# grospy/bitcoincashplus

Measured on AMD Instinct MI355X. Metric: equihash_200_9_solutions_per_sec, higher is better.
Workload: dtype uint32; 1 GPU; model=Equihash(200,9) mainnet PoW solver (BLAKE2b, K=9 collision rounds), global_batch=96, seq_len=2097152, parallelism=dp1 (nonce-space), solvers_in_flight=2, full=False, verified_solutions=0, gpu_cpu_verifier_disagreements=0, rows_dropped_all_nonces=231487, pairs_dropped_all_nonces=346475, candidates_dropped_all_nonces=0

## Files before the change

csrc/kernels/equihash_layout.h:

```cpp
#ifndef BCP_KERNELS_EQUIHASH_LAYOUT_H
#define BCP_KERNELS_EQUIHASH_LAYOUT_H

#include <cstddef>
#include <cstdint>
#include <stdexcept>

#if defined(__HIPCC__)
#define BCP_EH_HD __host__ __device__
#else
#define BCP_EH_HD
#endif

#ifndef BCP_EH_GEN_HPT
#define BCP_EH_GEN_HPT 2
#endif
#ifndef BCP_EH_GEN_NT
#define BCP_EH_GEN_NT 512
#endif
#ifndef BCP_EH_PRUNE_FROM
#define BCP_EH_PRUNE_FROM 9
#endif
#ifndef BCP_EH_MP_LATE
#define BCP_EH_MP_LATE 1
#endif
// ... 17 lines not shown
static_assert(BCP_EH_OVL >= 1 && BCP_EH_OVL <= 128, "the overflow list is walked by the first BCP_EH_OVL lanes");

namespace bcpk {

template <class C> constexpr int round_nt(int stage, bool carry);
template <class C> constexpr int round_mp(int stage, bool carry = false);
template <class C> constexpr bool round_prunes(int stage, bool carry = false);
template <class C> constexpr bool slot_round_fits(int stage);

template <int N_, int K_, int BB_, int CAP_, int NT_, int GENWG_, int NTG_, int MAXCAND_, int CAP4_ = CAP_,
          int CAP3_ = CAP_, int WGCU_ = 1, int GNT_ = 512, int GHPT_ = 2, int CAPF_ = 0, int MPX_ = 0, int GW_ = 0>
struct EhCfg {
    static constexpr int N = N_, K = K_;
    static constexpr int DB = N / (K + 1);
    static constexpr int BB = BB_;
    static constexpr int RB = DB - BB_;
    static constexpr int NB = 1 << BB_;
    static constexpr int NRESTS = 1 << RB;
    static constexpr int CAP = CAP_;
    static constexpr int CAPF = CAPF_ > 0 ? CAPF_ : CAP3_;
    static constexpr int MPX = MPX_;
    static constexpr int cap(int round) {
        return round == K_ ? CAPF : words(round - 1) >= 5 ? CAP_ : words(round - 1) == 4 ? CAP4_ : CAP3_;
    }
    static constexpr int AREA_NF = CAP_ > CAP4_ ? (CAP_ > CAP3_ ? CAP_ : CAP3_) : (CAP4_ > CAP3_ ? CAP4_ : CAP3_);
    static constexpr int AREA = AREA_NF > CAPF ? AREA_NF : CAPF;
    static constexpr int NT = NT_;
    static constexpr int NW = NT_ / 64;
    static constexpr int GW = GW_;
    static constexpr int RNT = NT_ - 64 * GW_;
    static constexpr int WGCU = WGCU_;
    static constexpr int LDS_BUDGET = 160 * 1024 / WGCU_;
    static constexpr int INIT = 1 << (DB + 1);
    static constexpr int GENWG = GENWG_;
    static constexpr int NTG = NTG_;
    static constexpr int GNT = GNT_, GHPT = GHPT_;
    static constexpr int RPW = INIT / GENWG_;
    static constexpr int IPH = 512 / N;
    static constexpr int NBYTES = N / 8;
    static constexpr int MAXCAND = MAXCAND_;
    static constexpr int L = 1 << K;
    static constexpr int bits(int stage) { return N - stage * DB - BB_; }
    static constexpr int words(int stage) { return (bits(stage) + 31) / 32; }
    static constexpr int WMAX = words(0);
    static constexpr int IB = AREA <= 4096 ? 12 : 13;
    static constexpr int DH = 16 - IB;
    static constexpr uint32_t DHM = (1u << DH) - 1;
    static constexpr int DX = 2 * DH;
    static constexpr int DR = BB_ > DX ? BB_ - DX : 0;
    static constexpr uint32_t RMASK = (1u << DR) - 1;
    static constexpr uint32_t IMASK = ((1u << IB) - 1) * 0x10001u;
    static constexpr bool cp(int stage) {
        return stage >= 1 && stage < K && 32 * words(stage) - bits(stage) >= DR;
    }
    static constexpr int pad(int stage) { return 32 * words(stage) - bits(stage); }
    static constexpr bool tp(int stage) {
        return BCP_EH_TABLE_PARENTS && stage >= 1 && stage <= K - 2 && !round_prunes<EhCfg>(stage + 1) &&
               !round_prunes<EhCfg>(stage + 1, true) && pad(stage) >= BB;
    }
    static constexpr int ptab(int stage) {
        const int a = round_mp<EhCfg>(stage, false) * round_nt<EhCfg>(stage, false);
        const int b = GW_ > 0 ? round_mp<EhCfg>(stage, true) * round_nt<EhCfg>(stage, true) : 0;
        return a > b ? a : b;
    }
    static constexpr uint32_t tpmask(int stage) { return (1u << (pad(stage) > BB ? BB + 1 : BB)) - 1; }
    static constexpr uint32_t rmask(int stage) { return tp(stage) ? (uint32_t)NB - 1 : cp(stage) ? RMASK : 0u; }
    static constexpr int sw(int stage) {
        return stage == 0 || tp(stage) ? words(stage) : words(stage) + (cp(stage) ? 1 : 2);
    }
    static constexpr size_t ROWS = (size_t)NB * AREA;
    static constexpr int ks(int stage) {
        return BCP_EH_KEY_SLOTS && stage >= 1 && stage < K && NRESTS >= 256 && slot_round_fits<EhCfg>(stage)
                   ? BCP_EH_KEY_SLOTS
                   : 0;
    }
    static constexpr int PDW = 2 * K + 2 + (BCP_EH_KEY_SLOTS ? 2 * K : 0);
    static constexpr bool H16 = NB > 512;
    static constexpr int HW = H16 ? NB / 2 : NB;
    static_assert(RPW * GENWG_ == INIT && RPW < 65535, "generation split");
    static_assert(RB > 0 && DB < 32, "digit geometry");
    static_assert(AREA < (1 << IB), "LDS row indices in parent words and signatures");
    static_assert(NT_ % 64 == 0 && NT_ <= 1024 && (NB <= NT_ || NB % NT_ == 0) && NB <= NTG_ && NT_ / 64 <= 64,
                  "workgroup shape");
    static_assert(words(K - 1) == 1, "final round keeps whole rows in one LDS word");
    static_assert(GW_ == 0 || (WGCU_ == 1 && RNT >= 128 && (NB <= RNT || NB % RNT == 0)), "carrying workgroup shape");
};

#ifndef BCP_EH_CAPF
#define BCP_EH_CAPF 6016
#endif
using Cfg200_9 = EhCfg<200, 9, 9, 4416, 1024, 512, 1024, 256, 4864, 5120, 1, BCP_EH_GEN_NT, BCP_EH_GEN_HPT, BCP_EH_CAPF, 0, BCP_EH_GW>;
using Cfg96_5 = EhCfg<96, 5, 7, 1280, 256, 256, 256, 256, 1280, 1280, 1, 512, 2, 0, 1, 1>;
using Cfg48_5 = EhCfg<48, 5, 3, 512, 64, 8, 64, 256>;

constexpr uint32_t NIL = 0xffffffffu;

template <class C, int NTG, int HPT> struct GenReg {
    static constexpr int RPT = HPT * C::IPH;
    static constexpr int RPW = NTG > 0 ? NTG * RPT : 1;
    static constexpr bool OK = NTG > 0 && C::INIT % RPW == 0;
    static constexpr int GWG = OK ? C::INIT / RPW : 1;
};

BCP_EH_HD inline __attribute__((always_inline)) uint64_t pack_tri(uint32_t d, uint32_t i, uint32_t j) {
    return ((uint64_t)d << 32) | (j << 16) | i;
}
template <class C> BCP_EH_HD inline __attribute__((always_inline)) uint32_t cpack(uint32_t d, uint32_t i, uint32_t j) {
    return i | (j << 16) | ((d & C::DHM) << C::IB) | (((d >> C::DH) & C::DHM) << (16 + C::IB));
}
template <class C> BCP_EH_HD inline __attribute__((always_inline)) uint32_t cunpack_d(uint32_t pw, uint32_t lastword) {
    return ((pw >> C::IB) & C::DHM) | (((pw >> (16 + C::IB)) & C::DHM) << C::DH) | ((lastword & C::RMASK) << C::DX);
}

template <class C> constexpr int un_walk_bend(int cap) { return (cap * 2 + 3) / 4 * 4; }
template <class C> constexpr int un_walk_list(int cap) { return un_walk_bend<C>(cap) + C::NRESTS * 4; }
template <class C> constexpr int round_nt(int stage, bool carry) { return carry && stage < C::K ? C::RNT : C::NT; }
template <class C> constexpr int round_mp(int stage, bool carry) {
    const int nt = round_nt<C>(stage, carry);
    return stage == C::K ? 1
                         : (C::AREA_NF + nt - 1) / nt + C::MPX +
                               (C::K == 9 && stage >= BCP_EH_MP_LATE_FROM ? BCP_EH_MP_LATE : 0);
}
template <class C> constexpr int round_un(int stage, bool carry = false) {
    const int cap = C::cap(stage);
    if (stage == C::K) return un_walk_list<C>(cap);
    const int pairs = round_mp<C>(stage, carry) * round_nt<C>(stage, carry) * 4;
    const int walk = un_walk_list<C>(cap) + pairs;
    return walk > pairs ? walk : pairs;
}
template <class C> constexpr int round_lds(int stage, bool prune, bool carry = false) {
    const int WR = C::words(stage - 1);
    const int WI = WR;
    const int cap = C::cap(stage);
    const int pruneb = prune ? cap * 4 + (C::cp(stage - 1) ? 0 : (cap * 2 + 3) / 4 * 4) : 0;
    const int hists = stage == C::K ? 0 : 2 * C::HW * 4 + (C::NB * (C::H16 ? 2 : 4) + 3) / 4 * 4;
    const int gen = carry ? 2 * C::NB * 4 + 16 * 8 : 0;
    return (cap * WI + 3) / 4 * 16 + pruneb + 4 + round_un<C>(stage, carry) + hists +
           (round_nt<C>(stage, carry) / 64 + 1) * 4 + gen;
}
template <class C> constexpr int un_slot_bend() { return C::NRESTS * 8 * 2; }
template <class C> constexpr int un_slot_ovl() { return un_slot_bend<C>() + C::NRESTS * 4; }
template <class C> constexpr int un_slot_list() { return un_slot_ovl<C>() + BCP_EH_OVL * 4; }
template <class C> constexpr int slot_un(int stage, bool carry = false) {
    return un_slot_list<C>() + round_mp<C>(stage, carry) * round_nt<C>(stage, carry) * 4;
}
template <class C> constexpr int slot_lds(int stage, bool prune, bool carry = false) {
    const int b = round_lds<C>(stage, prune, carry) - round_un<C>(stage, carry) + slot_un<C>(stage, carry) + 4;
    return carry ? (b + 7) / 8 * 8 : b;
}
struct EhBars {
    int n, list, filter, scan, sort;
};
constexpr EhBars eh_bars(bool slot) { return slot ? EhBars{7, 2, 3, 4, 6} : EhBars{10, 5, 6, 7, 9}; }
template <class C> constexpr bool round_prunes(int stage, bool carry) {
    constexpr int from = C::K == 9 ? BCP_EH_PRUNE_FROM : 2;
    return (stage >= from || stage == C::K) && stage >= 2 && round_lds<C>(stage, true, carry) <= C::LDS_BUDGET;
}

template <class C> constexpr bool slot_round_fits(int stage) {
    return slot_lds<C>(stage, round_prunes<C>(stage, false), false) <= C::LDS_BUDGET &&
           (C::GW == 0 || slot_lds<C>(stage, round_prunes<C>(stage, true), true) <= C::LDS_BUDGET);
}

template <class C> struct GenCarry {
    static constexpr int GT = C::GW > 0 ? 64 * C::GW : 64;
    static constexpr int NHASH = (C::INIT + C::IPH - 1) / C::IPH;
    static constexpr int ITERS = (C::K - 1) * C::NB;
    static constexpr int HB = ((NHASH + ITERS - 1) / ITERS + GT - 1) / GT;
    static constexpr int CH = HB * GT;
    static constexpr int RPT = HB * C::IPH;
    static constexpr int BPT = (C::NB + GT - 1) / GT;
    static_assert((long long)CH * ITERS >= NHASH, "the carrying rounds cover every hash");
};

template <class C> BCP_EH_HD inline uint64_t slot_parent(int stage, const uint32_t* slot) {
    const uint32_t* q = slot + C::words(stage);
    if (C::cp(stage)) return ((uint64_t)cunpack_d<C>(q[0], q[-1]) << 32) | (q[0] & C::IMASK);
    return ((uint64_t)q[1] << 32) | q[0];
}
template <class C>
BCP_EH_HD inline uint64_t table_parent(int stage, const uint32_t* row, uint32_t area, uint32_t pos,
                                       const uint32_t* btab_of_nonce, const uint32_t* ptab_of_nonce, bool* in_range) {
    const uint32_t d = row[C::words(stage) - 1] & C::tpmask(stage);
    const uint32_t o = d < (uint32_t)C::NB ? pos - btab_of_nonce[(size_t)d * C::NB + area] : NIL;
    *in_range = d < (uint32_t)C::NB && o < (uint32_t)C::ptab(stage);
    return ((uint64_t)d << 32) | (*in_range ? ptab_of_nonce[(size_t)d * C::ptab(stage) + o] : NIL);
}

}

namespace bcp {
namespace gpu {

template <class F> static void dispatch_cfg(unsigned n, unsigned k, F&& f) {
    if (n == 200 && k == 9) f(bcpk::Cfg200_9{});
    else if (n == 96 && k == 5) f(bcpk::Cfg96_5{});
    else if (n == 48 && k == 5) f(bcpk::Cfg48_5{});
    else throw std::invalid_argument("EquihashGpuSolver: unsupported (N,K); GPU supports (200,9),(96,5),(48,5)");
}

}
}

#endif
```

csrc/kernels/equihash_solver.hip:

```cpp
#include <hip/hip_runtime.h>

#include "crypto/hashes.h"
#include "kernels/blake2b_device.h"
#include "kernels/equihash_layout.h"
#include "kernels/equihash_pow.h"
#include "kernels/gpu_api.h"
#include "kernels/hip_util.h"

#include <algorithm>
#include <cstdlib>
#include <cstring>
#include <stdexcept>
#include <utility>

#ifndef BCP_EH_XCD_MAP
#define BCP_EH_XCD_MAP 1
#endif
#ifndef BCP_EH_PF_SLICES
#define BCP_EH_PF_SLICES 3
#endif
#ifndef BCP_EH_SLOT_LIST
#define BCP_EH_SLOT_LIST 1
#endif
#ifndef BCP_EH_SLOT_RB
#define BCP_EH_SLOT_RB 5
#endif
#ifndef BCP_EH_SLOT_RD
#define BCP_EH_SLOT_RD 10
#endif
#ifndef BCP_EH_GROUPS_DEFAULT
#define BCP_EH_GROUPS_DEFAULT(batch) ((batch) >= 48 ? (batch) / 24 : 1)
#endif

namespace bcpk {

constexpr uint32_t OOB = 0x80000000u;
typedef uint32_t u2v __attribute__((ext_vector_type(2)));
typedef uint32_t u3v __attribute__((ext_vector_type(3)));
typedef uint32_t u4v __attribute__((ext_vector_type(4)));

template <int CTRL, int ROWMASK = 0xf>
__device__ __forceinline__ uint32_t dpp0(uint32_t x) {
    return (uint32_t)__builtin_amdgcn_update_dpp(0, (int)x, CTRL, ROWMASK, 0xf, false);
}
template <bool MAX> __device__ __forceinline__ uint32_t wave_incl(uint32_t x) {
    auto op = [](uint32_t a, uint32_t b) -> uint32_t { return MAX ? (a > b ? a : b) : a + b; };
    x = op(x, dpp0<0x111>(x));
    x = op(x, dpp0<0x112>(x));
    x = op(x, dpp0<0x114>(x));
    x = op(x, dpp0<0x118>(x));
    x = op(x, dpp0<0x142, 0xa>(x));
    x = op(x, dpp0<0x143, 0xc>(x));
    return x;
}

template <int NT, int MAXPER = 4, class TS = uint32_t, class TD = TS>
__device__ uint32_t block_exscan(const TS* src, TD* dst, int n, uint32_t* wsum, uint32_t* mine = nullptr) {
    constexpr int NW = NT / 64;
    const int tid = threadIdx.x, lane = tid & 63;
    const int wid = __builtin_amdgcn_readfirstlane(tid >> 6);
    const int per = (n + NT - 1) / NT;
    uint32_t local[MAXPER];
    uint32_t s = 0;
#pragma unroll
    for (int q = 0; q < MAXPER; ++q) {
        const int i = tid * per + q;
        local[q] = (q < per && i < n) ? (uint32_t)src[i] : 0u;
        s += local[q];
    }
    const uint32_t x = wave_incl<false>(s);
    if (NW > 1) {
        if (lane == 63) wsum[wid] = x;
        __syncthreads();
    }
    const uint32_t wt = (NW > 1 && lane < NW) ? wsum[lane] : 0u;
    const uint32_t ws = wave_incl<false>(wt);
    const uint32_t before = NW > 1 ? __builtin_amdgcn_readlane(ws, wid) - __builtin_amdgcn_readlane(wt, wid) : 0u;
    const uint32_t total = NW > 1 ? __builtin_amdgcn_readlane(ws, NW - 1) : __builtin_amdgcn_readlane(x, 63);
    uint32_t base = before + x - s;
    if (mine) *mine = base;
#pragma unroll
    for (int q = 0; q < MAXPER; ++q) {
        const int i = tid * per + q;
        if (q < per && i < n) dst[i] = (TD)base;
        base += local[q];
    }
    __syncthreads();
    return total;
}
template <int NT, int MAXPER = 4, class T = uint32_t>
__device__ uint32_t block_exscan(T* v, int n, uint32_t* wsum) {
    return block_exscan<NT, MAXPER, T, T>(v, v, n, wsum);
}

template <int NT, int MAXPER = 4, class T = uint32_t>
__device__ void block_maxscan(T* v, int n, uint32_t* wsum) {
    constexpr int NW = NT / 64;
    const int tid = threadIdx.x, lane = tid & 63;
    const int wid = __builtin_amdgcn_readfirstlane(tid >> 6);
    const int per = (n + NT - 1) / NT;
    uint32_t local[MAXPER];
    uint32_t s = 0;
#pragma unroll
    for (int q = 0; q < MAXPER; ++q) {
        const int i = tid * per + q;
        local[q] = (q < per && i < n) ? (uint32_t)v[i] : 0u;
        s = max(s, local[q]);
    }
    const uint32_t x = wave_incl<true>(s);
    const uint32_t excl = dpp0<0x138>(x);
    if (NW > 1) {
        if (lane == 63) wsum[wid] = x;
        __syncthreads();
    }
    const uint32_t wt = (NW > 1 && lane < NW) ? wsum[lane] : 0u;
    const uint32_t ws = wave_incl<true>(wt);
    const uint32_t before = (NW > 1 && wid > 0) ? __builtin_amdgcn_readlane(ws, wid - 1) : 0u;
    uint32_t run = max(before, excl);
#pragma unroll
    for (int q = 0; q < MAXPER; ++q) {
        const int i = tid * per + q;
        run = max(run, local[q]);
        if (q < per && i < n) v[i] = (T)run;
    }
    __syncthreads();
}

template <int W> __device__ __forceinline__ void row_store(__amdgpu_buffer_rsrc_t rs, uint32_t off, const uint32_t* v) {
    if constexpr (W >= 4) {
        const u4v x = {v[0], v[1], v[2], v[3]};
        __builtin_amdgcn_raw_buffer_store_b128(x, rs, off, 0, 0);
        row_store<W - 4>(rs, off + 16, v + 4);
    } else if constexpr (W == 3) {
        const u3v x = {v[0], v[1], v[2]};
        __builtin_amdgcn_raw_buffer_store_b96(x, rs, off, 0, 0);
    } else if constexpr (W == 2) {
        const u2v x = {v[0], v[1]};
        __builtin_amdgcn_raw_buffer_store_b64(x, rs, off, 0, 0);
    } else if constexpr (W == 1) {
        __builtin_amdgcn_raw_buffer_store_b32(v[0], rs, off, 0, 0);
    }
}

template <int W> __device__ __forceinline__ void row_load(__amdgpu_buffer_rsrc_t rs, uint32_t off, uint32_t* v) {
    if constexpr (W >= 4) {
        const u4v x = __builtin_amdgcn_raw_buffer_load_b128(rs, off, 0, 0);
        v[0] = x.x, v[1] = x.y, v[2] = x.z, v[3] = x.w;
        row_load<W - 4>(rs, off + 16, v + 4);
    } else if constexpr (W == 3) {
        const u3v x = __builtin_amdgcn_raw_buffer_load_b96(rs, off, 0, 0);
        v[0] = x.x, v[1] = x.y, v[2] = x.z;
    } else if constexpr (W == 2) {
        const u2v x = __builtin_amdgcn_raw_buffer_load_b64(rs, off, 0, 0);
        v[0] = x.x, v[1] = x.y;
    } else if constexpr (W == 1) {
        v[0] = __builtin_amdgcn_raw_buffer_load_b32(rs, off, 0, 0);
    }
}

template <int WI> __device__ __forceinline__ void lds_row_xor(const uint32_t* rows, uint32_t i, uint32_t j, uint32_t* x) {
    if constexpr (WI % 2 == 0) {
        const u2v* r2 = reinterpret_cast<const u2v*>(rows);
#pragma unroll
        for (int w = 0; w < WI / 2; ++w) {
            const u2v a = r2[i * (WI / 2) + w], b = r2[j * (WI / 2) + w];
            x[2 * w] = a.x ^ b.x;
            x[2 * w + 1] = a.y ^ b.y;
        }
    } else {
#pragma unroll
        for (int w = 0; w < WI; ++w) x[w] = rows[i * WI + w] ^ rows[j * WI + w];
    }
}

__device__ __forceinline__ __amdgpu_buffer_rsrc_t buf_rsrc(const void* p, uint32_t bytes) {
    return __builtin_amdgcn_make_buffer_rsrc(const_cast<void*>(p), 0, bytes, 0x00020000);
}

constexpr int NXCD = 8;
template <int NB> __device__ __forceinline__ int xcd_bucket(int b, int it, int G, int nbk) {
    const int nonces = nbk / NB;
// ... 64 lines not shown
    const auto rs = buf_rsrc(R + (size_t)nonce * C::ROWS * SW0, (uint32_t)(C::ROWS * SW0 * 4));
    uint32_t* leaf = LEAF + (size_t)nonce * C::ROWS;
    for (int t = tid; t < C::RPW; t += NTG) {
        const uint32_t li = perm[t], d = dst[li];
        const uint32_t pos = base[d] + (uint32_t)t;
        if (pos < OCAP) {
            uint32_t o[W0];
#pragma unroll
            for (int w = 0; w < W0; ++w) o[w] = rows[li * W0 + w];
            const uint32_t slot = d * C::AREA + pos;
            row_store<SW0>(rs, slot * (SW0 * 4), o);
            leaf[slot] = r0 + li;
        }
    }
}

template <class C, bool HDR, int NTG, int HPT>
__global__ __launch_bounds__(NTG) __attribute__((amdgpu_waves_per_eu(1))) void eh_gen_reg(const EhBaseState* __restrict__ states, uint32_t* __restrict__ R,
                                                  uint32_t* __restrict__ LEAF, uint32_t* __restrict__ CTR0, int items) {
    using G = GenReg<C, NTG, HPT>;
    static_assert(G::OK, "register generation geometry");
    constexpr int W0 = C::words(0);
    constexpr int SW = (C::N + 31) / 32 + 1;
    constexpr uint32_t OCAP = C::cap(1);
    __shared__ uint32_t hist[C::NB], base[C::NB];
    __shared__ uint64_t r0p[HDR ? 16 : 1];
    const int tid = threadIdx.x;
    for (int b = blockIdx.x; b < items; b += gridDim.x) {
    int gw = b % G::GWG;
    int nonce = b / G::GWG;
    if (BCP_EH_XCD_MAP && (items / G::GWG) % NXCD == 0 && gridDim.x % NXCD == 0) {
        const int x = b % NXCD, j = b / NXCD;
        gw = j % G::GWG;
        nonce = x + NXCD * (j / G::GWG);
    }
    if (b != (int)blockIdx.x) __syncthreads();
    const EhBaseState& bs = states[nonce];
    for (int i = tid; i < C::NB; i += NTG) hist[i] = 0;
    if constexpr (HDR) {
        if (tid == 0) {
            uint64_t P[16];
            eh_hdr_round0_uniform(bs, P);
#pragma unroll
            for (int i = 0; i < 16; ++i) r0p[i] = P[i];
        }
    }
    __syncthreads();
    const uint32_t r0 = (uint32_t)gw * G::RPW;
    const uint32_t g0 = r0 / C::IPH;
    uint32_t rw[G::RPT][W0];
    uint32_t rk[G::RPT];
#pragma unroll
    for (int hh = 0; hh < HPT; ++hh) {
        const uint32_t g = g0 + hh * NTG + tid;
        uint64_t h[8];
        if constexpr (HDR) {
            uint64_t P[16];
#pragma unroll
            for (int i = 0; i < 16; ++i) P[i] = r0p[i];
            eh_hash_g_hdr_from(P, bs, g, h);
        } else {
            eh_hash_g(bs, g, h);
        }
#pragma unroll
        for (int s = 0; s < C::IPH; ++s) {
            uint32_t S[SW];
#pragma unroll
            for (int w = 0; w < SW; ++w) {
                uint32_t v = 0;
#pragma unroll
                for (int t = 0; t < 4; ++t) {
                    const int k = 4 * w + t;
                    v = (v << 8) | ((k < C::NBYTES) ? digest_byte(h, s * C::NBYTES + k) : 0u);
                }
                S[w] = v;
            }
            const int q = hh * C::IPH + s;
            const uint32_t d = S[0] >> (32 - C::BB);
#pragma unroll
            for (int w = 0; w < W0; ++w) rw[q][w] = (S[w] << C::BB) | (S[w + 1] >> (32 - C::BB));
            rk[q] = (atomicAdd(&hist[d], 1u) << 16) | d;
        }
    }
    __syncthreads();
    for (int b = tid; b < C::NB; b += NTG) {
        const uint32_t c = hist[b];
        base[b] = c ? atomicAdd(&CTR0[(size_t)nonce * C::NB + b], c) : 0u;
    }
    __syncthreads();
    constexpr int SW0 = C::sw(0);
    const auto rs = buf_rsrc(R + (size_t)nonce * C::ROWS * SW0, (uint32_t)(C::ROWS * SW0 * 4));
    const auto rl = buf_rsrc(LEAF + (size_t)nonce * C::ROWS, (uint32_t)(C::ROWS * 4));
#pragma unroll
    for (int q = 0; q < G::RPT; ++q) {
        const uint32_t d = rk[q] & 0xffff;
        const uint32_t pos = base[d] + (rk[q] >> 16);
        const uint32_t slot = d * C::AREA + pos;
        const bool ok = pos < OCAP;
        const uint32_t g = g0 + (q / C::IPH) * NTG + tid;
        const uint32_t li = g * C::IPH + (q % C::IPH);
        row_store<W0>(rs, ok ? slot * (SW0 * 4) : OOB, rw[q]);
        __builtin_amdgcn_raw_buffer_store_b32(li, rl, ok ? slot * 4 : OOB, 0, 0);
    }
    }
}

#define EH_STAMP(k)                                                                                  \
    do {                                                                                             \
        if constexpr (STAMP) {                                                                       \
            if (threadIdx.x == 0) stamps[(size_t)bk * 16 + (k)] = __builtin_amdgcn_s_memtime();        \
        }                                                                                            \
    } while (0)

struct EhCarry {
    const EhBaseState* states;
    uint32_t* R0;
    uint32_t* LEAF;
    uint32_t* CTR0;
    int nonces;
};

constexpr int EH_SCAN_BARS = 2;
template <int K, int NBAR> __device__ __forceinline__ void eh_bar() {
    static_assert(K >= 1 && K <= NBAR, "barrier outside the bucket iteration's count");
    __syncthreads();
}
#define EH_BAR_SCAN(k, nbar) static_assert((k) >= 1 && (k) + EH_SCAN_BARS - 1 <= (nbar), "scan barriers")

template <class C, int STAGE>
__device__ __forceinline__ void eh_carry_gen(const EhCarry& cy, int nbk, uint32_t* ghist, uint32_t* gbase, uint64_t* gr0p) {
    using GC = GenCarry<C>;
    constexpr int W0 = C::words(0);
    constexpr int SW = (C::N + 31) / 32 + 1;
    constexpr int SW0 = C::sw(0);
    constexpr int GT = GC::GT, HB = GC::HB;
    constexpr uint32_t OCAP = C::cap(1);
    const int gtid = (int)threadIdx.x - C::RNT;
    const int G = gridDim.x;
    auto chunk_of = [&](int b) -> int {
        const int nonce = b / C::NB, c = (STAGE - 1) * C::NB + b % C::NB;
        return (nonce < cy.nonces && (long long)c * GC::CH < GC::NHASH) ? c : -1;
    };
    auto prefix = [&](int b) {
        if (gtid == 0 && b / C::NB < cy.nonces) {
            uint64_t P[16];
            eh_hdr_round0_uniform(cy.states[b / C::NB], P);
#pragma unroll
            for (int i = 0; i < 16; ++i) gr0p[i] = P[i];
        }
    };
    constexpr bool SLOT = C::ks(STAGE) > 0;
    constexpr EhBars BAR = eh_bars(SLOT);
    constexpr int NBAR = BAR.n;
    constexpr int RA = 3, RB = SLOT ? BCP_EH_SLOT_RB : 5, RC = SLOT ? RB : 6, RD = SLOT ? BCP_EH_SLOT_RD : 10;
    static_assert(RA <= RB && RB <= RC && RC <= RD && RD <= 12, "BLAKE2b slices in order");
    EhHdrHash hs[HB];
    auto start = [&](int b) {
        const int c = chunk_of(b);
        if (c < 0) return;
        const EhBaseState& bs = cy.states[b / C::NB];
        uint64_t P[16];
#pragma unroll
        for (int i = 0; i < 16; ++i) P[i] = gr0p[i];
#pragma unroll
        for (int hh = 0; hh < HB; ++hh) {
            hs[hh].begin(P, bs, (uint32_t)c * GC::CH + (uint32_t)(hh * GT + gtid));
            hs[hh].template rounds<1, RA>(bs);
        }
    };
    int it = 0;
    int bk = xcd_bucket<C::NB>(blockIdx.x, 0, G, nbk);
    for (int i = gtid; i < C::NB; i += GT) ghist[i] = 0;
    prefix(bk);
    __syncthreads();
    start(bk);
    for (;;) {
        const int nonce = bk / C::NB;
        const int chunk = chunk_of(bk);
        const bool act = chunk >= 0;
        const EhBaseState& bs = cy.states[act ? nonce : 0];
        const int bn = xcd_bucket<C::NB>(blockIdx.x, it + 1, G, nbk);
        const bool more = bn >= 0;
        const uint32_t g0 = (uint32_t)chunk * GC::CH + (uint32_t)gtid;
        uint32_t rw[GC::RPT][W0];
        uint32_t rk[GC::RPT];
        uint32_t myb[GC::BPT];
        if (act) {
#pragma unroll
            for (int hh = 0; hh < HB; ++hh) hs[hh].template rounds<RA, RB>(bs);
        }
        eh_bar<1, NBAR>();
        if constexpr (!SLOT) {
            eh_bar<2, NBAR>();
            eh_bar<3, NBAR>();
            if (act) {
#pragma unroll
                for (int hh = 0; hh < HB; ++hh) hs[hh].template rounds<RB, RC>(bs);
            }
            eh_bar<4, NBAR>();
        }
        if (act) {
#pragma unroll
            for (int hh = 0; hh < HB; ++hh) hs[hh].template rounds<RC, RD>(bs);
        }
        if (more && bn / C::NB != nonce) prefix(bn);
        eh_bar<BAR.list, NBAR>();
        if (act) {
#pragma unroll
            for (int hh = 0; hh < HB; ++hh) {
                hs[hh].template rounds<RD, 12>(bs);
                uint64_t h[8];
                hs[hh].finish(bs, h);
                const uint32_t g = g0 + hh * GT;
#pragma unroll
                for (int s = 0; s < C::IPH; ++s) {
                    uint32_t S[SW];
#pragma unroll
                    for (int w = 0; w < SW; ++w) {
                        uint32_t v = 0;
#pragma unroll
                        for (int t = 0; t < 4; ++t) {
                            const int k = 4 * w + t;
                            v = (v << 8) | ((k < C::NBYTES) ? digest_byte(h, s * C::NBYTES + k) : 0u);
                        }
                        S[w] = v;
                    }
                    const int q = hh * C::IPH + s;
                    const uint32_t d = S[0] >> (32 - C::BB);
#pragma unroll
                    for (int w = 0; w < W0; ++w) rw[q][w] = (S[w] << C::BB) | (S[w + 1] >> (32 - C::BB));
                    rk[q] = NIL;
                    if (g * C::IPH + s < (uint32_t)C::INIT) rk[q] = (atomicAdd(&ghist[d], 1u) << 16) | d;
                }
            }
        }
        eh_bar<BAR.filter, NBAR>();
        if (act) {
#pragma unroll
            for (int k = 0; k < GC::BPT; ++k) {
                const int b = gtid + k * GT;
                const uint32_t c = b < C::NB ? ghist[b] : 0u;
                myb[k] = 0;
                if (c) myb[k] = atomicAdd(&cy.CTR0[(size_t)nonce * C::NB + b], c);
            }
        }
        eh_bar<BAR.scan, NBAR>();
        if (act)
            for (int i = gtid; i < C::NB; i += GT) ghist[i] = 0;
        eh_bar<BAR.scan + 1, NBAR>();
        if (act) {
#pragma unroll
            for (int k = 0; k < GC::BPT; ++k) {
                const int b = gtid + k * GT;
                if (b < C::NB) gbase[b] = myb[k];
            }
        }
        eh_bar<BAR.sort, NBAR>();
        if (act) {
            const auto rs = buf_rsrc(cy.R0 + (size_t)nonce * C::ROWS * SW0, (uint32_t)(C::ROWS * SW0 * 4));
            const auto rl = buf_rsrc(cy.LEAF + (size_t)nonce * C::ROWS, (uint32_t)(C::ROWS * 4));
#pragma unroll
            for (int q = 0; q < GC::RPT; ++q) {
                const uint32_t d = rk[q] & 0xffff;
                const uint32_t pos = gbase[d < (uint32_t)C::NB ? d : 0] + (rk[q] >> 16);
                const uint32_t slot = d * C::AREA + pos;
                const bool ok = rk[q] != NIL && pos < OCAP;
                const uint32_t li = (g0 + (q / C::IPH) * GT) * C::IPH + (q % C::IPH);
                row_store<W0>(rs, ok ? slot * (SW0 * 4) : OOB, rw[q]);
                __builtin_amdgcn_raw_buffer_store_b32(li, rl, ok ? slot * 4 : OOB, 0, 0);
            }
        }
        if (more) start(bn);
        eh_bar<NBAR, NBAR>();
        if (!more) break;
        bk = bn;
        ++it;
    }
}

template <class C, int STAGE, bool STAMP, bool CARRY = false>
__global__ __launch_bounds__(C::NT) __attribute__((amdgpu_waves_per_eu(C::WGCU * C::NT / 256)))
void eh_round(const uint32_t* __restrict__ Rin, const uint32_t* __restrict__ CTRin, uint32_t* __restrict__ Rout,
              uint32_t* __restrict__ CTRout, uint32_t* __restrict__ Pout, uint32_t* __restrict__ Bout,
              uint32_t* __restrict__ ncand, uint64_t* __restrict__ cand, uint64_t* __restrict__ stamps,
              uint32_t* __restrict__ pdrop, int nbk, EhCarry carry) {
    constexpr int WI = C::words(STAGE - 1);
    constexpr int WO = (STAGE < C::K) ? C::words(STAGE) : 1;
    constexpr int CAP = C::cap(STAGE);
    constexpr bool FINAL = STAGE == C::K;
    constexpr int PDW = C::PDW;
    static_assert(!CARRY || (C::GW > 0 && !FINAL && !STAMP), "only plain collision rounds carry generation");
    constexpr bool PRUNE = round_prunes<C>(STAGE, CARRY);
    static_assert(PRUNE == round_prunes<C>(STAGE), "a carrying round prunes like the plain one");
    constexpr bool SLOT = C::ks(STAGE) > 0;
    constexpr EhBars BAR = eh_bars(SLOT);
    constexpr int NBAR = BAR.n;
    constexpr int OVL = BCP_EH_OVL;
    static_assert((SLOT ? slot_lds<C>(STAGE, PRUNE, CARRY) : round_lds<C>(STAGE, PRUNE, CARRY)) <= 160 * 1024 / C::WGCU,
                  "round LDS budget");
    constexpr int NT = round_nt<C>(STAGE, CARRY);
    static_assert(!CARRY || NT / 64 > 1, "block_exscan runs its two barriers only with more than one wave");
    constexpr int RPL = (CAP + NT - 1) / NT;
    constexpr int MP = round_mp<C>(STAGE, CARRY);
    constexpr int SWI = C::sw(STAGE - 1);
    constexpr int SWO = STAGE < C::K ? C::sw(STAGE) : 1;
    constexpr bool TPO = !FINAL && C::tp(STAGE);
    constexpr int PTW = TPO ? C::ptab(STAGE) : 1;
// ... 137 lines not shown
        return __builtin_amdgcn_raw_buffer_load_b32(ctr_rs, b >= 0 ? (uint32_t)b * 4 : OOB, 0, 0);
    };

    for (;;) {
        const int nonce = bk / C::NB, d = bk % C::NB;
        EH_STAMP(0);
        if (tid == 0 && fill > (uint32_t)CAP) atomicAdd(&pdrop[nonce * PDW + C::K + STAGE], fill - CAP);
        {
            const uint32_t ot = opaque_tid();
#pragma unroll
            for (int u = 0; u < RPL; ++u) {
                const uint32_t r = ot + u * NT;
                if (r < n) {
                    if constexpr (WI % 2 == 0) {
#pragma unroll
                        for (int w = 0; w < WI; w += 2)
                            *reinterpret_cast<u2v*>(&rows[r * WI + w]) = u2v{nr[u][w], nr[u][w + 1]};
                    } else {
#pragma unroll
                        for (int w = 0; w < WI; ++w) rows[r * WI + w] = nr[u][w];
                    }
                    if constexpr (PRUNE) {
                        psig[r] = nr[u][WI];
                        if constexpr (!CPI) pdw[r] = (uint16_t)nr[u][WI + 1];
                    }
                    if constexpr (FOLD) {
                        const uint32_t key = nr[u][0] >> (32 - C::RB);
                        krank[u] = (key << 16) | atomicAdd(&bend[key], 1u);
                    }
                }
            }
            if constexpr (SLOT) {
#pragma unroll
                for (int u = 0; u < RPL; ++u) {
                    const uint32_t r = ot + u * NT;
                    if (r < n) {
                        const uint32_t key = krank[u] >> 16, t = krank[u] & 0xffff;
                        if (t < 8u) {
                            ktab[key * 8 + t] = (uint16_t)r;
                        } else {
                            const uint32_t o = atomicAdd(&novf, 1u);
                            if (o < (uint32_t)OVL) ovl[o] = (key << 16) | r;
                            krank[u] |= o < (uint32_t)OVL ? 0x4000u : 0x8000u;
                        }
                    }
                }
            }
        }
        if constexpr (!FINAL)
            for (int b = tid; b < C::HW; b += NT) hist_[b] = 0;
        if constexpr (!FOLD)
            for (int k = tid; k < C::NRESTS; k += NT) bend[k] = 0;
        if (tid == 0) npairs = 0;
        EH_STAMP(1);
        const int bn = xcd_bucket<C::NB>(blockIdx.x, it + 1, G, nbk);
        const bool more = bn >= 0;
        const uint32_t fn = more ? (uint32_t)__builtin_amdgcn_readfirstlane(fill_next) : 0u;
        const uint32_t nn = min(fn, (uint32_t)CAP);
        pf_bk = more ? bn : bk;
        pf_n = nn;
        const int bn2 = xcd_bucket<C::NB>(blockIdx.x, it + 2, G, nbk);
        issue(0, SLI);
        fill_next = fill_of(bn2);
        eh_bar<1, NBAR>();
        EH_STAMP(2);

        auto key_of = [&](uint32_t i) -> uint32_t { return rows[i * WI] >> (32 - C::RB); };
        uint32_t kpairs[FOLD ? RPL : 1];
        if constexpr (SLOT) {
            if constexpr (STAMP) {
                if (threadIdx.x == 0) stamps[(size_t)bk * 16 + 3] = stamps[(size_t)bk * 16 + 2];
            }
            issue(SLI, 2 * SLI);
        } else if constexpr (FOLD) {
            EH_BAR_SCAN(2, NBAR);
            block_exscan<NT, (C::NRESTS + NT - 1) / NT>(bend, C::NRESTS, wsum);
            const uint32_t ot = opaque_tid();
#pragma unroll
            for (int u = 0; u < RPL; ++u) {
                const uint32_t r = ot + u * NT;
                kpairs[u] = 0;
                if (r < n) {
                    const uint32_t key = krank[u] >> 16;
                    const uint32_t pos = bend[key] + (krank[u] & 0xffff);
                    const uint32_t e = key + 1 < (uint32_t)C::NRESTS ? bend[key + 1] : n;
                    sidx[pos] = (uint16_t)r;
                    krank[u] = pos;
                    kpairs[u] = min(e - pos - 1, 14u);
                    if (e - pos - 1 > 14u) atomicAdd(&pdrop[nonce * PDW + STAGE], e - pos - 1 - 14u);
                }
            }
        } else {
            for (uint32_t i = tid; i < n; i += NT) atomicAdd(&bend[key_of(i)], 1u);
            __syncthreads();
            block_exscan<NT, (C::NRESTS + NT - 1) / NT>(bend, C::NRESTS, wsum);
            for (uint32_t i = tid; i < n; i += NT) sidx[atomicAdd(&bend[key_of(i)], 1u)] = (uint16_t)i;
        }
        if constexpr (!SLOT) {
            issue(SLI, 2 * SLI);
            eh_bar<4, NBAR>();
            EH_STAMP(3);
        }

        if constexpr (FINAL) {
            static_assert(WI == 1, "final-round rows are one word");
            for (uint32_t p = tid; p < n; p += NT) {
                const uint32_t i = sidx[p], ri = rows[i], e = bend[ri >> (32 - C::RB)];
                for (uint32_t q = p + 1; q < e; ++q) {
                    const uint32_t j = sidx[q];
                    if ((rows[j] ^ ri) & ~RMI) continue;
                    if constexpr (PRUNE) {
                        if (shares_parent(i, j)) continue;
                    }
                    const uint32_t c = atomicAdd(&ncand[nonce], 1u);
                    if (c < (uint32_t)C::MAXCAND) cand[(size_t)nonce * C::MAXCAND + c] = pack_tri(d, i, j);
                }
            }
            issue(2 * SLI, RPL);
        } else {
            uint32_t cnt = 0;
            uint32_t le = 0, lm = 0, ln = 0;
            if constexpr (SLOT) {
                const uint32_t nov = __builtin_amdgcn_readfirstlane(novf);
                const uint32_t NO = min(nov, (uint32_t)OVL);
                const bool full = nov > (uint32_t)OVL;
                ovf_sum += nov;
                ovf_max = max(ovf_max, nov);
#pragma unroll
                for (int u = 0; u < RPL; ++u) {
                    kpairs[u] = 0;
                    if (tid + u * NT < n) {
                        const uint32_t t = krank[u] & 0x3fffu, f = krank[u] & 0xc000u;
                        kpairs[u] = f == 0x4000u ? 0u : min(t, 8u);
                        if (full && f) atomicAdd(&pdrop[nonce * PDW + STAGE], t - 8u);
                    }
                }
                if ((uint32_t)tid < NO) {
                    le = ovl[tid];
                    uint32_t m = 0;
                    for (uint32_t q = 0; q < (uint32_t)tid; ++q) m += (ovl[q] >> 16) == (le >> 16) ? 1u : 0u;
                    lm = min(m, 6u);
                    if (full) {
                        if (lm) atomicSub(&pdrop[nonce * PDW + STAGE], lm);
                    } else if (m > 6u) {
                        atomicAdd(&pdrop[nonce * PDW + STAGE], m - 6u);
                    }
                    ln = 8u + lm;
                    cnt = ln;
                }
            }
#pragma unroll
            for (int u = 0; u < RPL; ++u) cnt += kpairs[u];
            const uint32_t incl = wave_incl<false>(cnt);
            uint32_t wb = 0;
            if ((tid & 63) == 63) wb = atomicAdd(&npairs, incl);
            uint32_t o = __builtin_amdgcn_readlane(wb, 63) + incl - cnt;
            if constexpr (SLOT) {
                auto table_pairs = [&](uint32_t key, uint32_t c, uint32_t i) {
                    const u4v w = *reinterpret_cast<const u4v*>(&ktab[key * 8]);
                    const uint32_t room = o < (uint32_t)(MP * NT) ? (uint32_t)(MP * NT) - o : 0u;
                    const uint32_t ce = min(c, room);
                    if constexpr (BCP_EH_SLOT_LIST == 1) {
                        for (uint32_t q = 0; q < ce; ++q) {
                            const uint32_t ww = q < 4 ? (q < 2 ? w.x : w.y) : (q < 6 ? w.z : w.w);
                            plist[o + q] = ((q & 1) ? (ww & 0xffff0000u) : (ww << 16)) | i;
                        }
                    } else {
#pragma unroll
                        for (int q = 0; q < 8; ++q)
                            if ((uint32_t)q < ce) plist[o + q] = ((q & 1) ? (w[q >> 1] & 0xffff0000u) : (w[q >> 1] << 16)) | i;
                    }
                    o += c;
                };
#pragma unroll
                for (int u = 0; u < RPL; ++u)
                    if (kpairs[u]) table_pairs(krank[u] >> 16, kpairs[u], tid + u * NT);
                if (ln) {
                    const uint32_t i = le & 0xffffu;
                    table_pairs(le >> 16, 8u, i);
                    for (uint32_t q = 0, k = 0; q < (uint32_t)tid && k < lm; ++q) {
                        const uint32_t e = ovl[q];
                        if ((e >> 16) != (le >> 16)) continue;
                        if (o < (uint32_t)(MP * NT)) plist[o] = (e << 16) | i;
                        ++o, ++k;
                    }
                }
            } else {
#pragma unroll
            for (int u = 0; u < RPL; ++u) {
                if (!kpairs[u]) continue;
                const uint32_t p = krank[u];
                const uint32_t i = tid + u * NT;
                for (uint32_t q = p + 1; q <= p + kpairs[u]; ++q, ++o) {
                    if (o >= (uint32_t)(MP * NT)) continue;
                    plist[o] = ((uint32_t)sidx[q] << 16) | i;
                }
            }
            }
            eh_bar<BAR.list, NBAR>();
            EH_STAMP(7);
            const uint32_t P = npairs;
            const uint32_t Pc = min(P, (uint32_t)(MP * NT));
            if (tid == 0 && P > (uint32_t)(MP * NT)) atomicAdd(&pdrop[nonce * PDW + STAGE], P - MP * NT);
            uint32_t pv[MP], pd[MP];
#pragma unroll
            for (int u = 0; u < MP; ++u) {
                const uint32_t k = tid + u * NT;
                pv[u] = NIL;
                pd[u] = 0;
                if (k < Pc) {
                    const uint32_t pr = plist[k];
                    const uint32_t i = pr & 0xffff, j = pr >> 16;
                    uint32_t dest;
                    if (pair_keep(i, j, dest)) {
                        pv[u] = (j << 16) | i;
                        pd[u] = dest;
                        hinc(hist_, pd[u]);
                    }
                }
            }
            for (int k = tid; k < C::NRESTS; k += NT) bend[k] = 0;
            if constexpr (SLOT) {
                if (tid == 0) novf = 0;
            }
            eh_bar<BAR.filter, NBAR>();
            EH_STAMP(4);
            uint32_t myb[BPT];
#pragma unroll
            for (int k = 0; k < BPT; ++k) {
                const int b = tid * BPT + k;
                myb[k] = 0;
                if (b < C::NB) myb[k] = atomicAdd(&CTRout[(size_t)nonce * C::NB + b], hget(hist_, b));
            }
            issue(2 * SLI, RPL);
            uint32_t start = 0;
            uint32_t np;
            EH_BAR_SCAN(BAR.scan, NBAR);
            if constexpr (C::H16)
                np = block_exscan<NT, BPT, uint16_t, uint16_t>(reinterpret_cast<const uint16_t*>(hist_),
                                                               reinterpret_cast<uint16_t*>(cur_), C::NB, wsum, &start);
            else
                np = block_exscan<NT, BPT>(hist_, cur_, C::NB, wsum, &start);
#pragma unroll
            for (int u = 0; u < MP; ++u)
                if (pv[u] != NIL) spair[hinc(cur_, pd[u])] = pv[u];
#pragma unroll
            for (int k = 0; k < BPT; ++k) {
                const int b = tid * BPT + k;
                const uint32_t rb = myb[k] - start;
                if (b < C::NB) {
                    base[b] = (HT)rb;
                    start += hget(hist_, b);
                }
                if constexpr (TPO) {
                    const auto rs_b = buf_rsrc(Bout + ((size_t)nonce * C::NB + d) * C::NB, C::NB * 4);
                    __builtin_amdgcn_raw_buffer_store_b32(rb, rs_b, b < C::NB ? (uint32_t)b * 4 : OOB, 0, 0);
                }
            }
            eh_bar<BAR.sort, NBAR>();
            EH_STAMP(5);
            constexpr uint32_t OCAP = C::cap(STAGE + 1 <= C::K ? STAGE + 1 : C::K);
            constexpr uint32_t RMO = C::rmask(STAGE);
            const auto rs_out = buf_rsrc(Rout + (size_t)nonce * C::ROWS * SWO, (uint32_t)(C::ROWS * SWO * 4));
            const auto rs_p = buf_rsrc(Pout + (TPO ? ((size_t)nonce * C::NB + d) * PTW : 0), TPO ? PTW * 4 : 0);
#pragma unroll
            for (int u = 0; u < MP; ++u) {
                const uint32_t t = tid + u * NT;
                const uint32_t pr = t < np ? spair[t] : 0u;
                const uint32_t i = pr & 0xffff, j = pr >> 16;
                uint32_t x[WI + 1], o[WO];
                lds_row_xor<WI>(rows, i, j, x);
                x[WI - 1] &= ~RMI;
                x[WI] = 0;
                const uint32_t b = (x[0] >> (32 - C::DB)) & (C::NB - 1);
                const uint32_t pos = (HT)(base[b] + t);
                const bool ok = t < np && pos < OCAP;
                const uint32_t slot = b * C::AREA + pos;
#pragma unroll
                for (int w = 0; w < WO; ++w) o[w] = (x[w] << C::DB) | (x[w + 1] >> (32 - C::DB));
                uint32_t ov[SWO] = {};
#pragma unroll
                for (int w = 0; w < WO; ++w) ov[w] = o[w];
                if constexpr (TPO) {
                    ov[WO - 1] |= (uint32_t)d & RMO;
                } else if constexpr (C::cp(STAGE)) {
                    ov[WO - 1] |= (d >> C::DX) & RMO;
                    ov[WO] = cpack<C>(d, i, j);
                } else {
                    ov[WO] = (j << 16) | i;
                    ov[WO + 1] = d;
                }
                row_store<SWO>(rs_out, ok ? slot * (SWO * 4) : OOB, ov);
                if constexpr (TPO) __builtin_amdgcn_raw_buffer_store_b32(pr, rs_p, t < np ? t * 4 : OOB, 0, 0);
            }
        }
        eh_bar<NBAR, NBAR>();
        EH_STAMP(6);
        if constexpr (SLOT) {
            if (!more || bn / C::NB != nonce) {
                if (tid == 0 && ovf_sum) {
                    atomicAdd(&pdrop[nonce * PDW + 2 * C::K + 1 + STAGE], ovf_sum);
                    atomicMax(&pdrop[nonce * PDW + 3 * C::K + 1 + STAGE], ovf_max);
                }
                ovf_sum = ovf_max = 0;
            }
        }
        if (!more) break;
        bk = bn;
        ++it;
        fill = fn;
        n = nn;
    }
}


struct EhStages {
    const uint32_t* r[16];
    const uint32_t* p[16];
    const uint32_t* b[16];
};
template <class C>
__global__ __launch_bounds__(C::L < 64 ? 64 : C::L) void eh_expand(const uint32_t* __restrict__ LEAF, EhStages st,
                                                                  const uint32_t* __restrict__ ncand,
                                                                  const uint64_t* __restrict__ cand,
                                                                  uint32_t* __restrict__ out_idx,
                                                                  uint32_t* __restrict__ out_valid,
                                                                  uint32_t* __restrict__ nout,
                                                                  uint32_t* __restrict__ out_list) {
    constexpr int L = C::L;
    __shared__ uint32_t buf[2][L];
    __shared__ uint64_t tri[L / 2 > 0 ? L / 2 : 1];
    __shared__ uint32_t dup;
    const uint32_t c = blockIdx.x % C::MAXCAND;
    const uint32_t nonce = blockIdx.x / C::MAXCAND;
    const uint32_t t = threadIdx.x;
    const uint32_t nc = min(ncand[nonce], (uint32_t)C::MAXCAND);
    if (c >= nc) return;
    if (t == 0) {
        tri[0] = cand[(size_t)nonce * C::MAXCAND + c];
        dup = 0;
// ... 720 lines not shown
```

Measured before the change: 10410 Sol/s.

## Emit pair lists cooperatively per wave via head markers and max-scan

Adds a wave-cooperative pair-list builder. Each lane writes a packed head word (offset, key or sorted position, lane, unit) at the start of its pair run, then the wave fills the list with a max-prefix scan so every output slot is produced by one lane. This replaces the per-lane serial loops, which diverge badly when pair counts per row are uneven. It is on by default only for the sorted (non-slot) rounds. It costs an extra zeroing pass and scan, adds a per-wave capacity cap that may drop pairs, and exposes the sorted-round BLAKE2b slice split as macros.

```diff
diff --git a/csrc/kernels/equihash_layout.h b/csrc/kernels/equihash_layout.h
--- a/csrc/kernels/equihash_layout.h
+++ b/csrc/kernels/equihash_layout.h
@@ -193,6 +193,54 @@
     int n, list, filter, scan, sort;
 };
 constexpr EhBars eh_bars(bool slot) { return slot ? EhBars{7, 2, 3, 4, 6} : EhBars{10, 5, 6, 7, 9}; }
+template <class C> struct EhHead {
+    static constexpr int UB = 3, LB = 6;
+    static constexpr int KB = C::RB;
+    static constexpr int SLOT_OB = 32 - KB - LB - UB;
+    static constexpr int PB = 13;
+    static constexpr int SORT_OB = 32 - PB;
+    static constexpr uint32_t SLOT_OCAP = 1u << SLOT_OB;
+    static constexpr uint32_t SORT_OCAP = 1u << SORT_OB;
+    static constexpr int rpl_max() {
+        int m = 0;
+        for (int s = 1; s < C::K; ++s)
+            for (int c = 0; c <= (C::GW > 0 ? 1 : 0); ++c) {
+                const int nt = round_nt<C>(s, c != 0), r = (C::cap(s) + nt - 1) / nt;
+                m = r > m ? r : m;
+            }
+        return m;
+    }
+    static constexpr uint32_t SLOT_BLOCK_MAX = 64u * (8u * rpl_max() + 14u);
+    static constexpr uint32_t SORT_BLOCK_MAX = 64u * 14u * rpl_max();
+    static_assert(rpl_max() <= (1 << UB), "a lane's unit fits the head's unit bits");
+    static_assert(C::AREA_NF < (1 << PB), "a sorted position fits the head's position bits");
+    static_assert(SLOT_OB >= 12 && SLOT_OCAP % 64 == 0, "slot round: at least 4096 positions per wave block");
+    static_assert(SORT_BLOCK_MAX <= SORT_OCAP, "sorted round: no wave block passes the o_local range");
+};
+template <class C> BCP_EH_HD constexpr uint32_t head_slot(uint32_t o_local, uint32_t key, uint32_t lane, uint32_t unit) {
+    return (o_local << (32 - EhHead<C>::SLOT_OB)) | (key << (EhHead<C>::LB + EhHead<C>::UB)) | (lane << EhHead<C>::UB) | unit;
+}
+template <class C> BCP_EH_HD constexpr uint32_t head_slot_o(uint32_t h) { return h >> (32 - EhHead<C>::SLOT_OB); }
+template <class C> BCP_EH_HD constexpr uint32_t head_slot_key(uint32_t h) {
+    return (h >> (EhHead<C>::LB + EhHead<C>::UB)) & ((1u << EhHead<C>::KB) - 1);
+}
+template <class C> BCP_EH_HD constexpr uint32_t head_slot_row(uint32_t h, uint32_t wave, uint32_t nt) {
+    return wave * 64 + ((h >> EhHead<C>::UB) & 63u) + (h & ((1u << EhHead<C>::UB) - 1)) * nt;
+}
+template <class C> BCP_EH_HD constexpr uint32_t head_sorted(uint32_t o_local, uint32_t pos) { return (o_local << EhHead<C>::PB) | pos; }
+template <class C> BCP_EH_HD constexpr uint32_t head_sorted_o(uint32_t h) { return h >> EhHead<C>::PB; }
+template <class C> BCP_EH_HD constexpr uint32_t head_sorted_pos(uint32_t h) { return h & ((1u << EhHead<C>::PB) - 1); }
+static_assert(EhHead<Cfg200_9>::SLOT_OB == 12 && EhHead<Cfg96_5>::SLOT_OB == 14 && EhHead<Cfg48_5>::SLOT_OB == 18,
+              "o_local bits of a slot-round head");
+static_assert(EhHead<Cfg200_9>::SORT_OB == 19 && EhHead<Cfg96_5>::SORT_OB == 19 && EhHead<Cfg48_5>::SORT_OB == 19,
+              "o_local bits of a sorted-round head");
+static_assert(head_slot_o<Cfg200_9>(head_slot<Cfg200_9>(4095, 2047, 63, 7)) == 4095 &&
+                  head_slot_key<Cfg200_9>(head_slot<Cfg200_9>(4095, 2047, 63, 7)) == 2047 &&
+                  head_slot_row<Cfg200_9>(head_slot<Cfg200_9>(0, 0, 63, 7), 11, 768) == 11 * 64 + 63 + 7 * 768 &&
+                  head_sorted_pos<Cfg200_9>(head_sorted<Cfg200_9>(12543, 6015)) == 6015 &&
+                  head_sorted_o<Cfg200_9>(head_sorted<Cfg200_9>(12543, 6015)) == 12543,
+              "head fields do not overlap");
+
 template <class C> constexpr bool round_prunes(int stage, bool carry) {
     constexpr int from = C::K == 9 ? BCP_EH_PRUNE_FROM : 2;
     return (stage >= from || stage == C::K) && stage >= 2 && round_lds<C>(stage, true, carry) <= C::LDS_BUDGET;
diff --git a/csrc/kernels/equihash_solver.hip b/csrc/kernels/equihash_solver.hip
--- a/csrc/kernels/equihash_solver.hip
+++ b/csrc/kernels/equihash_solver.hip
@@ -22,11 +22,23 @@
 #ifndef BCP_EH_SLOT_LIST
 #define BCP_EH_SLOT_LIST 1
 #endif
+#ifndef BCP_EH_WAVE_LIST
+#define BCP_EH_WAVE_LIST 0
+#endif
+#ifndef BCP_EH_WAVE_LIST_SORTED
+#define BCP_EH_WAVE_LIST_SORTED 1
+#endif
 #ifndef BCP_EH_SLOT_RB
 #define BCP_EH_SLOT_RB 5
 #endif
 #ifndef BCP_EH_SLOT_RD
 #define BCP_EH_SLOT_RD 10
+#endif
+#ifndef BCP_EH_SORT_RC
+#define BCP_EH_SORT_RC 6
+#endif
+#ifndef BCP_EH_SORT_RD
+#define BCP_EH_SORT_RD 10
 #endif
 #ifndef BCP_EH_GROUPS_DEFAULT
 #define BCP_EH_GROUPS_DEFAULT(batch) ((batch) >= 48 ? (batch) / 24 : 1)
@@ -397,7 +409,7 @@
     constexpr bool SLOT = C::ks(STAGE) > 0;
     constexpr EhBars BAR = eh_bars(SLOT);
     constexpr int NBAR = BAR.n;
-    constexpr int RA = 3, RB = SLOT ? BCP_EH_SLOT_RB : 5, RC = SLOT ? RB : 6, RD = SLOT ? BCP_EH_SLOT_RD : 10;
+    constexpr int RA = 3, RB = SLOT ? BCP_EH_SLOT_RB : 5, RC = SLOT ? RB : BCP_EH_SORT_RC, RD = SLOT ? BCP_EH_SLOT_RD : BCP_EH_SORT_RD;
     static_assert(RA <= RB && RB <= RC && RC <= RD && RD <= 12, "BLAKE2b slices in order");
     EhHdrHash hs[HB];
     auto start = [&](int b) {
@@ -841,13 +853,66 @@
 #pragma unroll
             for (int u = 0; u < RPL; ++u) cnt += kpairs[u];
             const uint32_t incl = wave_incl<false>(cnt);
+            constexpr bool WLIST = SLOT ? BCP_EH_WAVE_LIST != 0 : BCP_EH_WAVE_LIST_SORTED != 0;
+            using HD = EhHead<C>;
+            constexpr uint32_t HOCAP = SLOT ? HD::SLOT_OCAP : HD::SORT_OCAP;
+            constexpr bool CAPPED = WLIST && (SLOT ? HD::SLOT_BLOCK_MAX : HD::SORT_BLOCK_MAX) > HOCAP;
             uint32_t wb = 0;
-            if ((tid & 63) == 63) wb = atomicAdd(&npairs, incl);
+            if constexpr (CAPPED) {
+                if ((tid & 63) == 63) {
+                    wb = atomicAdd(&npairs, min(incl, HOCAP));
+                    if (incl > HOCAP) atomicAdd(&pdrop[nonce * PDW + STAGE], incl - HOCAP);
+                }
+            } else {
+                if ((tid & 63) == 63) wb = atomicAdd(&npairs, incl);
+            }
             uint32_t o = __builtin_amdgcn_readlane(wb, 63) + incl - cnt;
+            uint32_t wlim = 0;
+            auto lim = [&]() -> uint32_t {
+                if constexpr (WLIST) return wlim;
+                else return (uint32_t)(MP * NT);
+            };
+            if constexpr (WLIST) {
+                const uint32_t lane = tid & 63;
+                const uint32_t wid = __builtin_amdgcn_readfirstlane(tid >> 6);
+                const uint32_t wbase = __builtin_amdgcn_readlane(wb, 63);
+                uint32_t wlen = __builtin_amdgcn_readlane(incl, 63);
+                if constexpr (CAPPED) wlen = min(wlen, HOCAP);
+                wlen = min(wlen, wbase < (uint32_t)(MP * NT) ? (uint32_t)(MP * NT) - wbase : 0u);
+                wlim = wbase + wlen;
+                uint32_t* blk = plist + wbase;
+                for (uint32_t k0 = 0; k0 < wlen; k0 += 64)
+                    if (k0 + lane < wlen) blk[k0 + lane] = 0;
+                uint32_t ol = incl - cnt;
+#pragma unroll
+                for (int u = 0; u < RPL; ++u) {
+                    if (kpairs[u] && ol < wlen) {
+                        if constexpr (SLOT) blk[ol] = head_slot<C>(ol, krank[u] >> 16, lane, u);
+                        else blk[ol] = head_sorted<C>(ol, krank[u]);
+                    }
+                    ol += kpairs[u];
+                }
+                o = wbase + ol;
+                uint32_t run = 0;
+                for (uint32_t k0 = 0; k0 < wlen; k0 += 64) {
+                    const uint32_t k = k0 + lane, kc = min(k, wlen - 1);
+                    const uint32_t h = max(wave_incl<true>(blk[kc]), run);
+                    run = __builtin_amdgcn_readlane(h, 63);
+                    uint32_t pr;
+                    if constexpr (SLOT) {
+                        const uint32_t q = kc - head_slot_o<C>(h);
+                        pr = ((uint32_t)ktab[head_slot_key<C>(h) * 8 + q] << 16) | head_slot_row<C>(h, wid, NT);
+                    } else {
+                        const uint32_t p = head_sorted_pos<C>(h), q = kc - head_sorted_o<C>(h);
+                        pr = ((uint32_t)sidx[p + 1 + q] << 16) | sidx[p];
+                    }
+                    if (k < wlen) blk[k] = pr;
+                }
+            }
             if constexpr (SLOT) {
                 auto table_pairs = [&](uint32_t key, uint32_t c, uint32_t i) {
                     const u4v w = *reinterpret_cast<const u4v*>(&ktab[key * 8]);
-                    const uint32_t room = o < (uint32_t)(MP * NT) ? (uint32_t)(MP * NT) - o : 0u;
+                    const uint32_t room = o < lim() ? lim() - o : 0u;
                     const uint32_t ce = min(c, room);
                     if constexpr (BCP_EH_SLOT_LIST == 1) {
                         for (uint32_t q = 0; q < ce; ++q) {
@@ -861,20 +926,22 @@
                     }
                     o += c;
                 };
-#pragma unroll
-                for (int u = 0; u < RPL; ++u)
-                    if (kpairs[u]) table_pairs(krank[u] >> 16, kpairs[u], tid + u * NT);
+                if constexpr (!WLIST) {
+#pragma unroll
+                    for (int u = 0; u < RPL; ++u)
+                        if (kpairs[u]) table_pairs(krank[u] >> 16, kpairs[u], tid + u * NT);
+                }
                 if (ln) {
                     const uint32_t i = le & 0xffffu;
                     table_pairs(le >> 16, 8u, i);
                     for (uint32_t q = 0, k = 0; q < (uint32_t)tid && k < lm; ++q) {
                         const uint32_t e = ovl[q];
                         if ((e >> 16) != (le >> 16)) continue;
-                        if (o < (uint32_t)(MP * NT)) plist[o] = (e << 16) | i;
+                        if (o < lim()) plist[o] = (e << 16) | i;
                         ++o, ++k;
                     }
                 }
-            } else {
+            } else if constexpr (!WLIST) {
 #pragma unroll
             for (int u = 0; u < RPL; ++u) {
                 if (!kpairs[u]) continue;
```

Result: no change. 10430 Sol/s (median of 6 runs) (+0.2%).
